# Eydcao/BSMS-GNN

Hardware: AMD Instinct MI355X
Metric: rollout steps/sec (1-step fwd+bwd) on airfoil mesh, batch=8 (higher is better)
Workload: dtype f32; 1 GPU; airfoil-like Delaunay mesh, 5233 nodes, 5 bi-stride levels, D=128, hidden_layer=3, batch 8 per GPU (global 8), consistent mesh; global_batch=8, parallelism=dp1, trainable_params=1917827

## Files before the change

### bsms-gnn_amd/build.py

```python
import hashlib
import os
import subprocess
import sys
from concurrent.futures import ThreadPoolExecutor

HERE = os.path.dirname(os.path.abspath(__file__))
CSRC = os.path.join(HERE, "csrc")
OBJ = os.path.join(HERE, "_build")
LIB = os.path.join(HERE, "libbsms_hip.so")
SOURCES = ["plan.hip", "rowsum.hip", "chain.hip", "chain_d32.hip", "chain_d64.hip", "chain_d96.hip", "chain_d128.hip", "chain_d160.hip", "chain_d192.hip", "chain_d224.hip",
           "chain_d256.hip", "efuse.hip", "efwd.hip", "wgrad.hip", "gmp.hip", "mlp.hip", "bsgmp.hip", "optim.hip", "hierarchy.hip", "sim.hip", "posgrad.hip", "batch.hip", "errsum.hip"]
HEADERS = ["common.h", "chain.h", "host_orch.h", "gmp_block.h", "chain_dev.h", "chain_kernels.h", "chain_edge.h", "chain_launch.h", os.path.join("..", "..", "include", "bsms_hip.h")]
FLAGS = ["--offload-arch=gfx950", "-O3", "-std=c++17", "-fPIC", "-Wall", "-Wno-unused-function"]
if os.environ.get("BSMS_EXPERIMENTS") == "1":
    FLAGS.append("-DBSMS_EXPERIMENTS")


def _hipcc():
    for c in (os.environ.get("HIPCC"), "/opt/rocm/bin/hipcc", "hipcc"):
        if c and (os.path.isabs(c) and os.path.exists(c) or not os.path.isabs(c)):
            return c
    raise RuntimeError("hipcc not found")


def _digest():
    h = hashlib.sha256((" ".join(FLAGS) + os.environ.get("BSMS_CHAIN_FLAGS", "")).encode())
    for f in SOURCES + HEADERS:
        with open(os.path.join(CSRC, f), "rb") as fh:
            h.update(fh.read())
    return h.hexdigest()


def build(force=False, verbose=True):
    os.makedirs(OBJ, exist_ok=True)
    stamp = os.path.join(OBJ, "stamp")
    digest = _digest()
    if not force and os.path.exists(LIB) and os.path.exists(stamp) and open(stamp).read() == digest:
        return LIB
    hipcc = _hipcc()

    def compile_one(src):
        obj = os.path.join(OBJ, os.path.basename(src).replace(".hip", ".o"))
        extra = ["-ffp-contract=off"] if src in ("rowsum.hip", "sim.hip", "batch.hip", "errsum.hip") else []
        if src.startswith("chain") and os.environ.get("BSMS_CHAIN_FLAGS"):
            extra += os.environ["BSMS_CHAIN_FLAGS"].split()
        cmd = [hipcc, *FLAGS, *extra, "-c", os.path.join(CSRC, src), "-o", obj]
        r = subprocess.run(cmd, capture_output=True, text=True)
        if r.returncode != 0:
            raise RuntimeError(f"hipcc failed on {src}:\n{r.stdout}\n{r.stderr}")
        if verbose and r.stderr.strip():
            print(r.stderr, file=sys.stderr)
        return obj

    with ThreadPoolExecutor(max_workers=len(SOURCES)) as ex:
        objs = list(ex.map(compile_one, SOURCES))
    r = subprocess.run([hipcc, "--offload-arch=gfx950", "-shared", "-fPIC", "-o", LIB, *objs], capture_output=True, text=True)
    if r.returncode != 0:
        raise RuntimeError(f"link failed:\n{r.stdout}\n{r.stderr}")
    with open(stamp, "w") as fh:
        fh.write(digest)
    if verbose:
        print(f"built {LIB} ({os.path.getsize(LIB) / 1e6:.1f} MB)")
    return LIB


# ... 44 lines not shown
```

### bsms-gnn_amd/csrc/chain.h

```cpp
#pragma once
#include "common.h"

namespace bsms {

constexpr int kMaxStages = 8;
constexpr int kComputeWaves = 4;
constexpr int kTileRows = kComputeWaves * 16;
constexpr int kChainThreads = (kComputeWaves + 1) * 64;
constexpr int kChainMaxThreads = 8 * 64;
constexpr int kChunkHdrFloats = 256;
constexpr size_t mask_words_per_row(int64_t D) { return size_t(4) * size_t((D + 127) / 128); }
constexpr int kPadRows = 2 * kTileRows;
constexpr size_t pad_rows(size_t rows) { return (rows + kPadRows - 1) / kPadRows * kPadRows + 2 * kPadRows; }
constexpr size_t act_floats(size_t rows, int64_t D) { return pad_rows(rows) * (size_t(D) + mask_words_per_row(D)); }
constexpr int fiber_ld(int64_t p) { return p + 1 <= 4 ? 4 : 8; }
constexpr int kScaleSlot = 255;
constexpr size_t pack_floats(int64_t D) { return size_t(D / 32) * (kChunkHdrFloats + size_t(D / 16) * 512); }

enum ChainIn { IN_ROWS = 0, IN_ROWS2 = 1, IN_SMALL = 2, IN_EDGE = 3 };
enum ChainOut { OUT_LN = 0, OUT_PLAIN = 1, OUT_SMALL = 2, OUT_PLAIN2 = 3 };
enum GradIn { G_ROWS_LN = 0, G_EDGE_LN = 1, G_SMALL = 2 };
enum GradFirst { F_NONE = 0, F_HEADS1 = 1, F_HEADS2 = 2 };

struct ChainFwdArgs {
  int64_t R;
  int ntiles;
  const float* x;
  const float* x2;
  int K0;
  const float* w0t;
  const float* bias_in;
  float* store_in;
  const int32_t *src, *dst;
  int32_t E, N;
  const float *Ps, *Pd;
  const float* pos;
  int64_t pos_bstride;
  int p;
  float* fiber_out;
  int nstage;
  const float4* wp[kMaxStages];
  const float4* wp0b;
  float* store[kMaxStages];
  float* y;
  float* y2;
  float* yln;
  float* rstd;
  const float* resid;
  const float* resid2;
  int accumulate;
  const float* wout;
  const float* bout;
  int C;
  unsigned long long* timing;
  int bf16;
  int store_mode;
  int out_mode;
  int nseq;
  const float4* wseq[kMaxStages + 2];
  int nload;
  int nring;
  float* amax[kMaxStages + 1];
};

struct ChainBwdArgs {
  int64_t R;
  int ntiles;
  const float* dy;
  const float* yln;
  const float* rstd;
  const int32_t* dst;
  int32_t E, N;
  const float* wout;
  int C;
  const float* mask_in;
  int nstage;
  const float4* wpt[kMaxStages];
  const float* mask[kMaxStages];
  float* gstore[kMaxStages + 1];
  const float4 *wh0, *wh1;
  float *dx, *dx2;
  const float* dres;
  int store_mode;
  int bf16;
  int nseq;
  const float4* wseq[kMaxStages + 2];
  int nload;
  int nring;
  float* gmax[kMaxStages + 1];
  int ablate;
};

enum PackKind { PACK_FRAG = 0, PACK_FRAG_T = 1, PACK_TRANSPOSE = 2, PACK_ROWS_BF16 = 3 };
struct PackDesc {
  const float* W;
  const float* bias;
  float* dst;
  int ld, row0, col0;
  int N, K;
  int kind;
  int bf16;
  int mate;
};
constexpr int kMaxPack = 40;
constexpr int kBoundWidth = 8192;
constexpr int kBoundSlots = 32;
struct PackTable {
  int n;
  PackDesc d[kMaxPack];
  float* zero;
};
int launch_prepack(const PackTable& t, hipStream_t s);

struct PackGroup {
  std::vector<PackDesc> descs;
  std::vector<float*> zeros;
  int biggest = 0;
  void* dev = nullptr;
  int device = -1;
};
void pack_group_append(PackGroup& g, const PackTable& t);
int launch_prepack_group(PackGroup& g, hipStream_t s);
int pack_group_open(bsms_pack_group_t* group, const char* who, PackGroup** g);

int launch_chain_fwd(int D, int in_mode, int out_mode, const ChainFwdArgs& a, hipStream_t s);
int launch_chain_bwd(int D, int gin_mode, int first_mode, const ChainBwdArgs& a, hipStream_t s);
template <int NB>
int launch_chain_fwd_nb(int in_mode, int out_mode, const ChainFwdArgs& a, hipStream_t s);
template <int NB>
int launch_chain_bwd_nb(int gin_mode, int first_mode, const ChainBwdArgs& a, hipStream_t s);

struct WgradJob {
  const float* G;
  const float* A;
  float* dW;
  float* db;
  int64_t R;
  int ldg, lda, ldw, col0;
  int bf16;
  const float *g_bound, *a_bound;
  float g_mul, a_mul;
// ... 82 lines not shown
```

### bsms-gnn_amd/csrc/chain_dev.h

```cpp
#pragma once
#include "chain.h"

using namespace bsms;

namespace {


using f32x4 = __attribute__((ext_vector_type(4))) float;
#ifndef BSMS_CHAIN_WPE
#define BSMS_CHAIN_WPE 4
#endif
constexpr int kPL = 2;


using f32x2 = __attribute__((ext_vector_type(2))) float;
using bf16x2 = __attribute__((ext_vector_type(2))) __bf16;
__device__ __forceinline__ unsigned pk_bf16(float lo, float hi) {
  const f32x2 v = {lo, hi};
  return __builtin_bit_cast(unsigned, __builtin_convertvector(v, bf16x2));
}
__device__ __forceinline__ float bf16_lo(unsigned u) { return __uint_as_float(u << 16); }
__device__ __forceinline__ float bf16_hi(unsigned u) { return __uint_as_float(u & 0xffff0000u); }

template <int NB>
// ... 129 lines not shown
      const int e = 32 * w + k;
      m = __builtin_amdgcn_alignbit(m, 0u - __float_as_uint(v[e >> 2][e & 3]), 31);
    }
    bits[w] = m;
  }
}

template <int NB>
__device__ __forceinline__ void load_features(f32x4 (&v)[NB], const float* vec, int g) {
  load_rows<NB>(v, vec, g);
}

__device__ __forceinline__ float group_sum(float s) {
  s += __shfl_xor(s, 16, 64);
  s += __shfl_xor(s, 32, 64);
  return s;
}

template <int NB>
__device__ __forceinline__ float row_sum(const f32x4 (&v)[NB]) {
  float s = 0.f;
#pragma unroll
  for (int t = 0; t < NB; ++t) s += (v[t][0] + v[t][1]) + (v[t][2] + v[t][3]);
  return group_sum(s);
}

template <int NB, int PL = kPL>
struct Ring {
  static constexpr int D = NB * 16;
  static constexpr int NCH = NB / 2;
  static constexpr int CHF = kChunkHdrFloats + NB * 256 * PL;
  static constexpr int CH4 = CHF / 4;
  static constexpr int PER = CHF / 256;
  static constexpr int SIDE_FLOATS = 8 * D;
  static constexpr int PRE_FLOATS = SIDE_FLOATS + 256;
  static constexpr int PRE4 = PRE_FLOATS / 4;
  static constexpr size_t lds_bytes(int nr) { return (size_t(PRE_FLOATS) + size_t(nr) * CHF) * sizeof(float); }
  static_assert(CHF % 256 == 0 && PER < 64, "chunk = whole LDS-DMA instructions, countable by vmcnt");
  static_assert(NB % 2 == 0, "K blocks are pairs of 16-feature blocks");
};

__device__ __forceinline__ void lds_barrier() { asm volatile("s_waitcnt lgkmcnt(0)\n\ts_barrier" ::: "memory"); }

__device__ __forceinline__ void glds16(const void* gsrc, unsigned lds_dst) {
  unsigned keep;
  asm volatile("s_mov_b32 %0, m0\n\ts_mov_b32 m0, %2\n\ts_nop 0\n\tglobal_load_lds_dwordx4 %1, off\n\ts_mov_b32 m0, %0"
               : "=&s"(keep) : "v"(gsrc), "s"(lds_dst) : "memory");
}

struct Slot { int i, nr; };

template <int NB, int PL, int NL, int LI>
__device__ __forceinline__ void loader_run(const float4* const* wseq, int nseq, float4* lds, int lane, int ntiles, int nr,
                                           const float* side = nullptr) {
  using R = Ring<NB, PL>;
  constexpr int MINE = (R::PER - LI + NL - 1) / NL;
  __builtin_amdgcn_s_setprio(3);
  const unsigned pre0 = __builtin_amdgcn_readfirstlane((unsigned)(uintptr_t)lds);
  const unsigned lds0 = pre0 + unsigned(R::PRE_FLOATS * sizeof(float));
  if (side) {
    if (LI == 0) {
      const unsigned dst = pre0;
#pragma unroll
      for (int i = 0; i < R::SIDE_FLOATS / 256; ++i) glds16(reinterpret_cast<const float4*>(side) + i * 64 + lane, dst + i * 1024);
    }
    asm volatile("s_waitcnt vmcnt(0)\n\ts_barrier" ::: "memory");
  }
  const int my_tiles = (ntiles - int(blockIdx.x) + int(gridDim.x) - 1) / int(gridDim.x);
  const int per_tile = nseq * R::NCH, total = my_tiles * per_tile;
  int is = 0, ic = 0, islot = 0;
  auto issue = [&]() {
    const float4* src = wseq[is] + size_t(ic) * R::CH4 + lane;
    const unsigned dst = lds0 + unsigned(islot) * unsigned(R::CHF * sizeof(float));
#pragma unroll
    for (int i = 0; i < MINE; ++i) glds16(src + (LI + i * NL) * 64, dst + (LI + i * NL) * 1024);
    if (++ic == R::NCH) { ic = 0; if (++is == nseq) is = 0; }
    if (++islot == nr) islot = 0;
  };
  const int ahead = nr - 1;
  for (int j = 0; j < ahead && j < total; ++j) issue();
  for (int j = 0; j < total; ++j) {
    const int younger = min(ahead - 1, total - 1 - j);
    switch (younger) {
      case 0: asm volatile("s_waitcnt vmcnt(0)" ::: "memory"); break;
      case 1: asm volatile("s_waitcnt vmcnt(%0)" ::"n"(MINE) : "memory"); break;
      case 2: asm volatile("s_waitcnt vmcnt(%0)" ::"n"(2 * MINE <= 63 ? 2 * MINE : 63) : "memory"); break;
      case 3: asm volatile("s_waitcnt vmcnt(%0)" ::"n"(3 * MINE <= 63 ? 3 * MINE : 63) : "memory"); break;
      default: asm volatile("s_waitcnt vmcnt(%0)" ::"n"(4 * MINE <= 63 ? 4 * MINE : 63) : "memory"); break;
    }
    asm volatile("s_barrier" ::: "memory");
    if (j + ahead < total) issue();
  }
}
template <int NB, int PL = kPL>
__device__ __forceinline__ void loader_dispatch(int nl, int li, const float4* const* wseq, int nseq, float4* lds, int lane, int ntiles,
                                                int nr, const float* side = nullptr) {
  if (nl == 1) loader_run<NB, PL, 1, 0>(wseq, nseq, lds, lane, ntiles, nr, side);
  else if (nl == 2) { if (li == 0) loader_run<NB, PL, 2, 0>(wseq, nseq, lds, lane, ntiles, nr, side); else loader_run<NB, PL, 2, 1>(wseq, nseq, lds, lane, ntiles, nr, side); }
  else { if (li == 0) loader_run<NB, PL, 3, 0>(wseq, nseq, lds, lane, ntiles, nr, side); else if (li == 1) loader_run<NB, PL, 3, 1>(wseq, nseq, lds, lane, ntiles, nr, side);
         else loader_run<NB, PL, 3, 2>(wseq, nseq, lds, lane, ntiles, nr, side); }
}

using u32x4 = __attribute__((ext_vector_type(4))) unsigned;
using bf16x8 = __attribute__((ext_vector_type(8))) __bf16;
using f16x8 = __attribute__((ext_vector_type(8))) _Float16;

template <int NB>
__device__ __forceinline__ void split_block(const f32x4 (&act)[NB], int kb2, float s, u32x4& bh, u32x4& bl) {
#pragma unroll
  for (int v = 0; v < 4; ++v) {
    unsigned h, l;
    split_h2(act[2 * kb2 + (v >> 1)][2 * (v & 1)], act[2 * kb2 + (v >> 1)][2 * (v & 1) + 1], s, h, l);
    bh[v] = h;
    bl[v] = l;
  }
}

template <int NB>
__device__ __forceinline__ void round_block(const f32x4 (&act)[NB], int kb2, u32x4& bh) {
#pragma unroll
  for (int v = 0; v < 4; ++v) bh[v] = pk_bf16(act[2 * kb2 + (v >> 1)][2 * (v & 1)], act[2 * kb2 + (v >> 1)][2 * (v & 1) + 1]);
}

__device__ __forceinline__ f32x4 mma_bf(const float4& a, const u32x4& b, f32x4 c) {
  return __builtin_amdgcn_mfma_f32_16x16x32_bf16(__builtin_bit_cast(bf16x8, a), __builtin_bit_cast(bf16x8, b), c, 0, 0, 0);
}
__device__ __forceinline__ f32x4 mma(const float4& a, const u32x4& b, f32x4 c) {
  return __builtin_amdgcn_mfma_f32_16x16x32_f16(__builtin_bit_cast(f16x8, a), __builtin_bit_cast(f16x8, b), c, 0, 0, 0);
}

template <int NB>
__device__ __forceinline__ float row_amax(const f32x4 (&v)[NB]) {
  float m = 0.f;
#pragma unroll
  for (int t = 0; t < NB; ++t) {
    m = fmaxf(fmaxf(m, fabsf(v[t][0])), fabsf(v[t][1]));
    m = fmaxf(fmaxf(m, fabsf(v[t][2])), fabsf(v[t][3]));
  }
  m = fmaxf(m, __shfl_xor(m, 16, 64));
  return fmaxf(m, __shfl_xor(m, 32, 64));
}

__device__ __forceinline__ bool any_slot(float* const (&slots)[kMaxStages + 1]) {
  bool any = false;
#pragma unroll
  for (int k = 0; k <= kMaxStages; ++k) any |= slots[k] != nullptr;
  return any;
}
template <int NB>
__device__ __forceinline__ unsigned* bound_row(float4* lds, int wave, int lane, bool wanted) {
  if (!wanted) return nullptr;
  unsigned* row = reinterpret_cast<unsigned*>(reinterpret_cast<float*>(lds) + Ring<NB>::SIDE_FLOATS) + wave * 16;
  if (lane < 16) row[lane] = 0u;
// ... 267 lines not shown
```

### bsms-gnn_amd/csrc/chain_edge.h

```cpp
#pragma once
#include "chain_dev.h"

namespace {

struct PairOff { unsigned a, b; };
template <int NB>
__device__ __forceinline__ PairOff pair_offsets(int64_t row, int lane) {
  constexpr int D = NB * 16;
  const bool hi = (lane & 8) != 0;
  const int64_t rowA = row - (lane & 8);
  return PairOff{unsigned((rowA * D + 4 * (lane >> 4) + (hi ? 16 : 0)) * 4), unsigned(((rowA + 8) * D + 4 * (lane >> 4) + (hi ? 0 : 16)) * 4)};
}
template <int NB>
__device__ __forceinline__ void store_pair_nt(const f32x4 (&v)[NB], float* base, PairOff off, int lane, int t) {
  using i32x4 = __attribute__((ext_vector_type(4))) int;
  const bool hi = (lane & 8) != 0;
  const i32x4 own = __builtin_bit_cast(i32x4, v[t + 1]);
  i32x4 got;
#pragma unroll
  for (int r = 0; r < 4; ++r) got[r] = __builtin_amdgcn_update_dpp(own[r], own[r], 0x128, 0xf, 0xf, false);
  const f32x4 x = __builtin_bit_cast(f32x4, got);
  const f32x4 dA = hi ? x : v[t], dB = hi ? v[t] : x;
  char* b = reinterpret_cast<char*>(base) + 64 * t;
  __builtin_nontemporal_store(dA, reinterpret_cast<f32x4*>(b + off.a));
// ... 179 lines not shown
    float4 f0 = body[0], f1 = body[2 * 64];
    if (c == 0) fw = int(__float_as_uint(reinterpret_cast<const float*>(cur)[kScaleSlot]) >> 23);
    const int cb = c & 1;
    int islot = 0;
    auto pair = [&](int t, int rb, const float4& a0, const float4& a1, const unsigned (&piece)[4], bool first) {
      acc[rb][t] = mma(a0, vec4(piece), (ZERO && first && c == 0) ? zero : acc[rb][t]);
      acc[rb][t + 1] = mma(a1, vec4(piece), (ZERO && first && c == 0) ? zero : acc[rb][t + 1]);
      const int s = (islot * NSTEP + NSLOT - 1) / NSLOT;
      if (s < NSTEP && s * NSLOT / NSTEP == islot)
        valu_step<NB, RB, SAVE, MASK>(s, c, act, pc, st, rs, mword, store_base, bits_base, off, moff, lane);
      ++islot;
      __builtin_amdgcn_sched_barrier(0);
    };
    __builtin_amdgcn_sched_barrier(0);
#pragma unroll
    for (int t = 0; t < NB; t += 2) {
      float4 n0 = body[(t * 2 + 1) * 64], n1 = body[(t * 2 + 3) * 64];
#pragma unroll
      for (int rb = 0; rb < RB; ++rb) pair(t, rb, f0, f1, pc[rb][cb].l, true);
#pragma unroll
      for (int rb = 0; rb < RB; ++rb) pair(t, rb, f0, f1, pc[rb][cb].h, false);
      f0 = n0;
      f1 = n1;
      if (t + 2 < NB) {
        n0 = body[((t + 2) * 2) * 64];
        n1 = body[((t + 2) * 2 + 2) * 64];
      }
#pragma unroll
      for (int rb = 0; rb < RB; ++rb) pair(t, rb, f0, f1, pc[rb][cb].h, false);
      f0 = n0;
      f1 = n1;
    }
    if (FIN != 0 && c == Rg::NCH - 1) {
#pragma unroll
      for (int rb = 0; rb < RB; ++rb) finish_stage<NB, FIN == 2>(acc[rb], rs[rb].E, fw, reinterpret_cast<const float*>(cur), lane);
    }
  }
}

template <int NB, int RB>
struct EdgeTile {
  static constexpr int rows = kTileRows * RB;
  static constexpr int waves_per_eu = (NB * RB <= 8) ? 4 : 2;
  static constexpr int resident = (NB * RB <= 8) ? 2 : 1;
};

template <int NB, int RB, int SAVE, bool LONE = false>
__global__ __launch_bounds__(kChainMaxThreads) __attribute__((amdgpu_waves_per_eu(LONE ? 2 : EdgeTile<NB, RB>::waves_per_eu)))
void k_edge_fwd(ChainFwdArgs a) {
  constexpr int D = NB * 16;
  extern __shared__ __attribute__((aligned(16))) float4 lds[];
  const int tid = threadIdx.x, lane = tid & 63, wave = tid >> 6, lg = lane >> 4;
  const int cw = int(blockDim.x >> 6) - a.nload, tile_rows = 16 * RB * cw;
  if (wave >= cw) {
    loader_dispatch<NB>(a.nload, wave - cw, a.wseq, a.nseq, lds, lane, a.ntiles, a.nring, a.w0t);
    return;
  }
  const float rcpE = 1.f / float(a.E);
  auto fetch_endpoints = [&](int tile, int (&i)[RB], int (&j)[RB], int (&b)[RB]) {
#pragma unroll
    for (int rb = 0; rb < RB; ++rb) {
      const int64_t r = int64_t(tile) * tile_rows + wave * (16 * RB) + rb * 16 + (lane & 15);
      const EdgeRef e = edge_ref(unsigned(r < a.R ? r : 0), unsigned(a.E), rcpE);
      i[rb] = a.src[e.q];
      j[rb] = a.dst[e.q];
      b[rb] = e.b;
    }
  };
  int ni[RB], nj[RB], nbat[RB];
  fetch_endpoints(blockIdx.x, ni, nj, nbat);
  lds_barrier();
  const float* w0t = reinterpret_cast<const float*>(lds);
  Slot slot{0, a.nring};
  float4* const ring = lds + Ring<NB>::PRE4;
  unsigned* brow = bound_row<NB>(lds, wave, lane, any_slot(a.amax));
  for (int tile = blockIdx.x; tile < a.ntiles; tile += gridDim.x) {
    int64_t row[RB];
    PairOff off[RB];
    unsigned moff[RB];
    f32x4 act[RB][NB], acc[RB][NB];
    float pi[RB][7], pj[RB][7];
#ifdef BSMS_EXPERIMENTS
    int stamp_i = 0;
    unsigned long long waited = 0;
    auto stamp = [&]() { if (a.timing && tid == 0 && stamp_i < 16) a.timing[int64_t(tile) * 16 + stamp_i++] = __builtin_amdgcn_s_memtime(); };
#else
    auto stamp = [] {};
#endif
    stamp();
#pragma unroll
    for (int rb = 0; rb < RB; ++rb) {
      row[rb] = int64_t(tile) * tile_rows + wave * (16 * RB) + rb * 16 + (lane & 15);
      off[rb] = pair_offsets<NB>(wave * (16 * RB) + rb * 16 + (lane & 15), lane);
      moff[rb] = unsigned(((wave * (16 * RB) + rb * 16 + (lane & 15)) * (4 * mask_words<NB>()) + lg * mask_words<NB>()) * 4);
      const int i = ni[rb], j = nj[rb], b = nbat[rb];
      load_rows<NB>(act[rb], a.Ps + (int64_t(b) * a.N + i) * D, lg);
      load_rows<NB>(acc[rb], a.Pd + (int64_t(b) * a.N + j) * D, lg);
      const float* pb = a.pos + b * a.pos_bstride;
      if (a.p == 2) {
        const float2 xi = *reinterpret_cast<const float2*>(pb + int64_t(i) * 2), xj = *reinterpret_cast<const float2*>(pb + int64_t(j) * 2);
        pi[rb][0] = xi.x; pi[rb][1] = xi.y; pj[rb][0] = xj.x; pj[rb][1] = xj.y;
#pragma unroll
        for (int c = 2; c < 7; ++c) pi[rb][c] = pj[rb][c] = 0.f;
      } else {
#pragma unroll
        for (int c = 0; c < 7; ++c) {
          const int cc = c < a.p ? c : 0;
          pi[rb][c] = pb[int64_t(i) * a.p + cc];
          pj[rb][c] = pb[int64_t(j) * a.p + cc];
        }
      }
    }
    if (tile + int(gridDim.x) < a.ntiles) fetch_endpoints(tile + gridDim.x, ni, nj, nbat);
    __builtin_amdgcn_sched_barrier(0);
    stamp();
#pragma unroll
    for (int rb = 0; rb < RB; ++rb) {
#pragma unroll
      for (int t = 0; t < NB; ++t) act[rb][t] += acc[rb][t];
      float n2 = 0.f;
#pragma unroll
      for (int c = 0; c < 7; ++c)
        if (c < a.p) {
          const float rel = pi[rb][c] - pj[rb][c];
          n2 = fmaf(rel, rel, n2);
          axpy_features<NB>(act[rb], w0t + c * D, rel, lg);
        }
      const float nrm = sqrtf(n2);
      axpy_features<NB>(act[rb], w0t + a.p * D, nrm, lg);
      relu_into<NB>(act[rb], act[rb]);
      if (a.fiber_out && row[rb] < a.R && lg == 0) {
        float f[8];
#pragma unroll
        for (int c = 0; c < 7; ++c) f[c] = c < a.p ? pi[rb][c] - pj[rb][c] : (c == a.p ? nrm : 0.f);
        f[7] = a.p == 7 ? nrm : 0.f;
        const int ld = fiber_ld(a.p);
        float4* dst = reinterpret_cast<float4*>(a.fiber_out + row[rb] * ld);
        dst[0] = make_float4(f[0], f[1], f[2], f[3]);
        if (ld == 8) dst[1] = make_float4(f[4], f[5], f[6], f[7]);
      }
    }
    float* pending = a.store_in;
    stamp();
    for (int l = 0; l < a.nstage; ++l) {
      float* st_tile = SAVE ? pending + int64_t(tile) * (tile_rows * D) : nullptr;
      unsigned* bits_tile = SAVE ? reinterpret_cast<unsigned*>(pending + pad_rows(a.R) * D) + int64_t(tile) * (tile_rows * 4 * mask_words<NB>()) : nullptr;
#ifdef BSMS_EXPERIMENTS
      stage_rb<NB, RB, SAVE, true, true, 2, LONE>(acc, act, ring, slot, lane, st_tile, bits_tile, off, moff, brow, l, nullptr, a.timing ? &waited : nullptr);
#else
      stage_rb<NB, RB, SAVE, true, true, 2, LONE>(acc, act, ring, slot, lane, st_tile, bits_tile, off, moff, brow, l);
#endif
      stamp();
      if (l + 1 < a.nstage) {
#pragma unroll
        for (int rb = 0; rb < RB; ++rb) relu_into<NB>(act[rb], acc[rb]);
        pending = a.store[l];
      }
    }
#pragma unroll
    for (int rb = 0; rb < RB; ++rb) {
      const float mean = row_sum<NB>(acc[rb]) * (1.f / D);
      float ss = 0.f;
#pragma unroll
      for (int t = 0; t < NB; ++t)
#pragma unroll
        for (int r = 0; r < 4; ++r) {
          acc[rb][t][r] -= mean;
          ss = fmaf(acc[rb][t][r], acc[rb][t][r], ss);
        }
      ss = group_sum(ss);
      const float rstd = 1.f / sqrtf(ss * (1.f / D) + 1e-5f);
#pragma unroll
      for (int t = 0; t < NB; ++t)
#pragma unroll
        for (int r = 0; r < 4; ++r) acc[rb][t][r] *= rstd;
      const int64_t roff = row[rb] < a.R ? row[rb] * D : -1;
      store_rows<NB, false>(acc[rb], a.yln, roff, lg);
      if (a.rstd && roff >= 0 && lg == 0) a.rstd[row[rb]] = rstd;
      store_rows<NB, false>(acc[rb], a.y, roff, lg, a.out_mode);
    }
    stamp();
#ifdef BSMS_EXPERIMENTS
    if (a.timing && tid == 0) a.timing[int64_t(tile) * 16 + 11] = waited;
#endif
  }
  if (SAVE) flush_bounds(a.amax, kMaxStages + 1, brow, wave, lane);
}

template <int NB, int RB, bool LONE = false, bool STORE = true>
__global__ __launch_bounds__(kChainMaxThreads) __attribute__((amdgpu_waves_per_eu(LONE ? 2 : EdgeTile<NB, RB>::waves_per_eu)))
void k_edge_bwd(ChainBwdArgs a) {
  constexpr int D = NB * 16, W = mask_words<NB>();
  extern __shared__ __attribute__((aligned(16))) float4 lds[];
  const int tid = threadIdx.x, lane = tid & 63, wave = tid >> 6, lg = lane >> 4;
  const int cw = int(blockDim.x >> 6) - a.nload, tile_rows = 16 * RB * cw;
  if (wave >= cw) {
    loader_dispatch<NB>(a.nload, wave - cw, a.wseq, a.nseq, lds, lane, a.ntiles, a.nring);
    return;
  }
  const float rcpE = 1.f / float(a.E);
  auto fetch_targets = [&](int tile, int64_t (&node)[RB]) {
#pragma unroll
    for (int rb = 0; rb < RB; ++rb) {
      const int64_t r = int64_t(tile) * tile_rows + wave * (16 * RB) + rb * 16 + (lane & 15);
      const EdgeRef e = edge_ref(unsigned(r < a.R ? r : 0), unsigned(a.E), rcpE);
      node[rb] = int64_t(e.b) * a.N + a.dst[e.q];
    }
  };
  int64_t nnode[RB];
  fetch_targets(blockIdx.x, nnode);
  Slot slot{0, a.nring};
  float4* const ring = lds + Ring<NB>::PRE4;
  unsigned* brow = bound_row<NB>(lds, wave, lane, any_slot(a.gmax));
  for (int tile = blockIdx.x; tile < a.ntiles; tile += gridDim.x) {
    int64_t row[RB], rowc[RB];
    PairOff off[RB];
    unsigned moff[RB];
    f32x4 g[RB][NB], acc[RB][NB];
    float rs[RB];
#pragma unroll
    for (int rb = 0; rb < RB; ++rb) {
      row[rb] = int64_t(tile) * tile_rows + wave * (16 * RB) + rb * 16 + (lane & 15);
      rowc[rb] = row[rb] < a.R ? row[rb] : 0;
      off[rb] = pair_offsets<NB>(wave * (16 * RB) + rb * 16 + (lane & 15), lane);
      moff[rb] = 0;
      load_rows<NB>(g[rb], a.dy + nnode[rb] * D, lg);
      load_rows<NB>(acc[rb], a.yln + rowc[rb] * D, lg);
      rs[rb] = a.rstd[rowc[rb]];
    }
    if (tile + int(gridDim.x) < a.ntiles) fetch_targets(tile + gridDim.x, nnode);
    __builtin_amdgcn_sched_barrier(0);
#pragma unroll
    for (int rb = 0; rb < RB; ++rb) {
      const float m1 = row_sum<NB>(g[rb]) * (1.f / D);
      float s2 = 0.f;
#pragma unroll
      for (int t = 0; t < NB; ++t)
#pragma unroll
        for (int r = 0; r < 4; ++r) s2 = fmaf(g[rb][t][r], acc[rb][t][r], s2);
      s2 = group_sum(s2);
      const float m2 = s2 * (1.f / D);
#pragma unroll
      for (int t = 0; t < NB; ++t)
#pragma unroll
        for (int r = 0; r < 4; ++r) g[rb][t][r] = rs[rb] * (g[rb][t][r] - m1 - acc[rb][t][r] * m2);
    }
    float* pending = a.gstore[0];
    for (int k = 0; k < a.nstage; ++k) {
      unsigned mbits[RB][W];
#pragma unroll
      for (int rb = 0; rb < RB; ++rb)
#pragma unroll
        for (int w = 0; w < W; ++w)
          mbits[rb][w] = reinterpret_cast<const unsigned*>(a.mask[k] + pad_rows(a.R) * D)[rowc[rb] * (4 * W) + lg * W + w];
#ifdef BSMS_EXPERIMENTS
      float* const gtile = STORE ? pending + int64_t(a.ablate ? 0 : tile) * (tile_rows * D) : nullptr;
#else
      float* const gtile = STORE ? pending + int64_t(tile) * (tile_rows * D) : nullptr;
#endif
      stage_rb<NB, RB, STORE ? 1 : 0, false, true, 1, LONE>(acc, g, ring, slot, lane, gtile, nullptr, off, moff, brow, k);
#pragma unroll
      for (int rb = 0; rb < RB; ++rb)
#pragma unroll
        for (int t = 0; t < NB; ++t)
#pragma unroll
          for (int r = 0; r < 4; ++r) {
            const int keep = __builtin_amdgcn_sbfe((int)mbits[rb][(4 * t + r) >> 5], (4 * t + r) & 31, 1);
            g[rb][t][r] = __uint_as_float(__float_as_uint(acc[rb][t][r]) & (unsigned)keep);
          }
      pending = a.gstore[k + 1];
    }
#pragma unroll
    for (int rb = 0; rb < RB; ++rb) {
      if (a.gmax[a.nstage]) note_amax(brow, a.nstage, row_amax<NB>(g[rb]), lane);
      store_rows<NB, false>(g[rb], pending, row[rb] < a.R ? row[rb] * D : -1, lg);
    }
  }
  flush_bounds(a.gmax, kMaxStages + 1, brow, wave, lane);
}

}
```

### bsms-gnn_amd/csrc/chain_launch.h

```cpp
#pragma once
#include <algorithm>
#include <cstdlib>

#include "chain_edge.h"
#include "chain_kernels.h"

namespace {

template <int NB>
constexpr int resident_per_cu() { return NB <= 4 ? 4 : NB == 8 ? 2 : 1; }

template <int NB>
int chain_compute_waves(int64_t R) {
  const int cus = device_cu_count();
  const int64_t slots = int64_t(cus) * resident_per_cu<NB>();
  if (resident_per_cu<NB>() >= 4 || ceil_div(R, kTileRows) <= slots) return kComputeWaves;
  const int64_t need = ceil_div(R, slots * 16);
  return need <= 7 ? (int)need : kComputeWaves;
}

template <int NB>
unsigned persistent_grid(int64_t ntiles) {
  const int cus = device_cu_count();
  return (unsigned)std::min<int64_t>(ntiles, int64_t(cus) * resident_per_cu<NB>());
}

inline int knob(const char* name, int dflt) {
#ifdef BSMS_EXPERIMENTS
  const char* e = getenv(name);
  return e ? atoi(e) : dflt;
#else
  (void)name;
  return dflt;
#endif
}

inline int edge_rb_mode() {
#ifdef BSMS_EXPERIMENTS
  static const int m = [] { const char* e = getenv("BSMS_EDGE_RB"); return e ? atoi(e) : -1; }();
  return m;
#else
  return -1;
#endif
}

template <int NB>
int edge_compute_waves() {
  static const int cw = NB >= 16 ? knob("BSMS_EDGE_CW16", 7) : knob("BSMS_EDGE_CW", 7);
  return cw;
}
template <int NB, int RB>
int pick_edge_waves(int64_t R) {
  const int fixed = edge_compute_waves<NB>();
#ifdef BSMS_EXPERIMENTS
  if (getenv(NB >= 16 ? "BSMS_EDGE_CW16" : "BSMS_EDGE_CW") || getenv("BSMS_EDGE_CW_FIXED")) return fixed;
#endif
  const double slope = (NB >= 16 ? 0.25 : 0.53) * RB;
  const int64_t slots = int64_t(device_cu_count()) * EdgeTile<NB, RB>::resident;
  auto cost_of = [&](int cw) {
    const int64_t tiles = ceil_div(R, int64_t(16) * RB * cw);
    const int64_t per = ceil_div(tiles, std::min<int64_t>(tiles, slots));
    return double(per) * (1.0 + slope * cw);
  };
  int best = fixed;
  double best_cost = cost_of(fixed) * 0.92;
  for (int cw = 6; cw >= 4; --cw) {
    const double cost = cost_of(cw);
    if (cost < best_cost * (1.0 - 1e-9)) { best_cost = cost; best = cw; }
  }
  return best;
}
template <int NB>
int edge_loader_waves() {
  static const int nl = NB >= 16 ? knob("BSMS_EDGE_NL16", 1) : knob("BSMS_EDGE_NL", 1);
  return nl;
}
inline int chain_loader_waves() {
  static const int nl = knob("BSMS_CHAIN_NL", 1);
  return nl;
}

template <int NB, int PL = kPL>
int max_ring() { return (int)std::min<size_t>(6, (size_t(160) * 1024 - Ring<NB, PL>::PRE_FLOATS * sizeof(float)) / (Ring<NB, PL>::CHF * sizeof(float))); }
template <int NB, int PL = kPL>
void pick_stream(int64_t ntiles, int cw, int nload_default, int& nload, int& nring) {
  static const int deep = knob("BSMS_RING_DEEP", 6), lone_nl = knob("BSMS_LONE_NL", 2), shared = knob("BSMS_RING", 3);
  nload = std::max(1, std::min(nload_default, 8 - cw));
  nring = std::min(shared, max_ring<NB, PL>());
  if (ntiles <= device_cu_count()) {
    nload = std::max(nload, std::min(lone_nl, 8 - cw));
    nring = std::min(deep, max_ring<NB, PL>());
  }
  const int mine = (Ring<NB, PL>::PER + nload - 1) / nload;
  while (nring > 3 && (nring - 2) * mine > 63) --nring;
}

template <int NB>
size_t ring_lds_max() { return Ring<NB>::lds_bytes(max_ring<NB>()); }

template <int NB, int RB, int SAVE>
int launch_edge_fwd_t(ChainFwdArgs& a, hipStream_t s) {
  const int cw = pick_edge_waves<NB, RB>(a.R);
  a.ntiles = (int)ceil_div(a.R, 16 * RB * cw);
  pick_stream<NB>(a.ntiles, cw, edge_loader_waves<NB>(), a.nload, a.nring);
  const unsigned grid = (unsigned)std::min<int64_t>(a.ntiles, int64_t(device_cu_count()) * EdgeTile<NB, RB>::resident);
  const unsigned threads = (cw + a.nload) * 64;
  const size_t lds = Ring<NB>::lds_bytes(a.nring);
  static const int lone = knob("BSMS_EDGE_LONE", 1);
  if (lone && a.ntiles <= device_cu_count() && !a.timing)
    return launch_dyn_lds<k_edge_fwd<NB, RB, SAVE, true>>("edge_fwd", "single-round build", grid, threads, lds, ring_lds_max<NB>(), a, s);
  return launch_dyn_lds<k_edge_fwd<NB, RB, SAVE>>("edge_fwd", nullptr, grid, threads, lds, ring_lds_max<NB>(), a, s);
}

template <int NB>
bool launch_edge_fwd(ChainFwdArgs& a, hipStream_t s, int& rc) {
  if (a.bf16 || a.nstage < 1 || a.store_mode != 1 || a.resid || a.resid2 || edge_rb_mode() == 0 || a.R >= (int64_t(1) << 31)) return false;
  const bool save = a.store_in != nullptr;
  for (int l = 0; l + 1 < a.nstage; ++l)
    if ((a.store[l] != nullptr) != save) return false;
  constexpr int RBIG = NB == 8 ? 2 : 1;
  const int64_t cus = device_cu_count(), rows1 = 16 * edge_compute_waves<NB>();
  bool big = RBIG == 2 && a.R >= cus * rows1 && ceil_div(a.R, rows1) <= cus * EdgeTile<NB, 1>::resident;
  if (edge_rb_mode() > 0) big = RBIG == 2 && edge_rb_mode() == 2;
  if (big) rc = save ? launch_edge_fwd_t<NB, RBIG, 1>(a, s) : launch_edge_fwd_t<NB, RBIG, 0>(a, s);
  else rc = save ? launch_edge_fwd_t<NB, 1, 1>(a, s) : launch_edge_fwd_t<NB, 1, 0>(a, s);
  return true;
}

template <int NB, int RB, bool STORE>
int launch_edge_bwd_t(ChainBwdArgs& a, hipStream_t s) {
  const int cw = pick_edge_waves<NB, RB>(a.R);
  a.ntiles = (int)ceil_div(a.R, 16 * RB * cw);
  pick_stream<NB>(a.ntiles, cw, edge_loader_waves<NB>(), a.nload, a.nring);
  const unsigned grid = (unsigned)std::min<int64_t>(a.ntiles, int64_t(device_cu_count()) * EdgeTile<NB, RB>::resident);
  const unsigned threads = (cw + a.nload) * 64;
  const size_t lds = Ring<NB>::lds_bytes(a.nring);
  static const int lone = knob("BSMS_EDGE_LONE", 1);
  if (lone && a.ntiles <= device_cu_count())
    return launch_dyn_lds<k_edge_bwd<NB, RB, true, STORE>>("edge_bwd", STORE ? "single-round build" : "single-round no-store build", grid, threads, lds, ring_lds_max<NB>(), a, s);
  return launch_dyn_lds<k_edge_bwd<NB, RB, false, STORE>>("edge_bwd", STORE ? nullptr : "no-store build", grid, threads, lds, ring_lds_max<NB>(), a, s);
}

template <int NB>
bool launch_edge_bwd(ChainBwdArgs& a, hipStream_t s, int& rc) {
  if (a.bf16 || a.nstage < 1 || a.store_mode != 1 || edge_rb_mode() == 0 || a.R >= (int64_t(1) << 31)) return false;
  if (!a.gstore[a.nstage]) return false;
  const bool store = a.gstore[0] != nullptr;
  for (int k = 0; k < a.nstage; ++k)
    if ((a.gstore[k] != nullptr) != store || !a.mask[k]) return false;
  constexpr int RBIG = NB == 8 ? 2 : 1;
  bool big = RBIG == 2 && a.R >= int64_t(device_cu_count()) * 16 * edge_compute_waves<NB>();
  if (edge_rb_mode() > 0) big = RBIG == 2 && edge_rb_mode() == 2;
  if (store) rc = big ? launch_edge_bwd_t<NB, RBIG, true>(a, s) : launch_edge_bwd_t<NB, 1, true>(a, s);
  else rc = big ? launch_edge_bwd_t<NB, RBIG, false>(a, s) : launch_edge_bwd_t<NB, 1, false>(a, s);
  return true;
}

template <int NB>
int bf_edge_waves(int64_t R) {
  static const int forced = knob("BSMS_BFEDGE_CW", 0);
  if (forced > 0) return forced;
  return R > int64_t(device_cu_count()) * resident_per_cu<NB>() * 16 * kComputeWaves ? 7 : kComputeWaves;
}

template <int NB, int IN, int OUT>
int launch_fwd_t(const ChainFwdArgs& a0, hipStream_t s) {
  ChainFwdArgs a = a0;
  a.nseq = 0;
  for (int l = 0; l < a.nstage; ++l) {
    a.wseq[a.nseq++] = a.wp[l];
    if (IN == IN_ROWS2 && l == 0) a.wseq[a.nseq++] = a.wp0b;
  }
  if constexpr ((NB == 8 || NB == 16) && IN == IN_EDGE && OUT == OUT_LN) {
    int rc = BSMS_OK;
    if (launch_edge_fwd<NB>(a, s, rc)) return rc;
  }
  if constexpr (NB == 8 && (IN == IN_ROWS || IN == IN_ROWS2 || IN == IN_SMALL)) {
    static const int fs_rows = knob("BSMS_FS_ROWS", kFsMaxRows);
    if (!a.bf16 && a.R <= fs_rows && a.nseq >= 1 && a.nseq <= kMaxStages + 1) {
      hipLaunchKernelGGL((k_fs_fwd<IN, OUT>), dim3((unsigned)ceil_div(a.R, 16)), dim3(256), 0, s, a);
      BSMS_LAUNCH_CHECK();
      return BSMS_OK;
    }
  }
  int cw = (IN == IN_EDGE) ? bf_edge_waves<NB>(a.R) : chain_compute_waves<NB>(a.R);
  a.ntiles = (int)ceil_div(a.R, 16 * cw);
  bool rows2_lone = false;
// ... 107 lines not shown
```

Before: 196.3 steps/s.

## Balance edge-kernel tail tiles across blocks by splitting leftover row blocks

Edge forward and backward kernels now map work in two parts: full rounds of tiles strided over the grid, plus a remainder of 16*RB-row blocks spread evenly across all blocks. Each block's leftover share runs with only some of its compute waves active, and the idle waves keep the ring barriers in step. This targets tail imbalance when the tile count is not a multiple of the resident slots. The wave-count cost model also changes to match the new mapping. The extra branching and the partial-wave barrier loop add complexity and risk of sync mismatch.

```diff
diff --git a/bsms-gnn_amd/build.py b/bsms-gnn_amd/build.py
--- a/bsms-gnn_amd/build.py
+++ b/bsms-gnn_amd/build.py
@@ -10,7 +10,7 @@
 LIB = os.path.join(HERE, "libbsms_hip.so")
 SOURCES = ["plan.hip", "rowsum.hip", "chain.hip", "chain_d32.hip", "chain_d64.hip", "chain_d96.hip", "chain_d128.hip", "chain_d160.hip", "chain_d192.hip", "chain_d224.hip",
            "chain_d256.hip", "efuse.hip", "efwd.hip", "wgrad.hip", "gmp.hip", "mlp.hip", "bsgmp.hip", "optim.hip", "hierarchy.hip", "sim.hip", "posgrad.hip", "batch.hip", "errsum.hip"]
-HEADERS = ["common.h", "chain.h", "host_orch.h", "gmp_block.h", "chain_dev.h", "chain_kernels.h", "chain_edge.h", "chain_launch.h", os.path.join("..", "..", "include", "bsms_hip.h")]
+HEADERS = ["common.h", "chain.h", "host_orch.h", "gmp_block.h", "chain_dev.h", "chain_kernels.h", "chain_edge.h", "chain_launch.h", "edge_balance.h", os.path.join("..", "..", "include", "bsms_hip.h")]
 FLAGS = ["--offload-arch=gfx950", "-O3", "-std=c++17", "-fPIC", "-Wall", "-Wno-unused-function"]
 if os.environ.get("BSMS_EXPERIMENTS") == "1":
     FLAGS.append("-DBSMS_EXPERIMENTS")
diff --git a/bsms-gnn_amd/csrc/chain.h b/bsms-gnn_amd/csrc/chain.h
--- a/bsms-gnn_amd/csrc/chain.h
+++ b/bsms-gnn_amd/csrc/chain.h
@@ -1,5 +1,6 @@
 #pragma once
 #include "common.h"
+#include "edge_balance.h"
 
 namespace bsms {
 
@@ -60,6 +61,7 @@
   const float4* wseq[kMaxStages + 2];
   int nload;
   int nring;
+  EdgeBalance bal;
   float* amax[kMaxStages + 1];
 };
 
@@ -87,6 +89,7 @@
   const float4* wseq[kMaxStages + 2];
   int nload;
   int nring;
+  EdgeBalance bal;
   float* gmax[kMaxStages + 1];
   int ablate;
 };
diff --git a/bsms-gnn_amd/csrc/chain_dev.h b/bsms-gnn_amd/csrc/chain_dev.h
--- a/bsms-gnn_amd/csrc/chain_dev.h
+++ b/bsms-gnn_amd/csrc/chain_dev.h
@@ -205,7 +205,7 @@
 
 template <int NB, int PL, int NL, int LI>
 __device__ __forceinline__ void loader_run(const float4* const* wseq, int nseq, float4* lds, int lane, int ntiles, int nr,
-                                           const float* side = nullptr) {
+                                           const float* side = nullptr, int given_tiles = -1) {
   using R = Ring<NB, PL>;
   constexpr int MINE = (R::PER - LI + NL - 1) / NL;
   __builtin_amdgcn_s_setprio(3);
@@ -219,7 +219,7 @@
     }
     asm volatile("s_waitcnt vmcnt(0)\n\ts_barrier" ::: "memory");
   }
-  const int my_tiles = (ntiles - int(blockIdx.x) + int(gridDim.x) - 1) / int(gridDim.x);
+  const int my_tiles = given_tiles >= 0 ? given_tiles : (ntiles - int(blockIdx.x) + int(gridDim.x) - 1) / int(gridDim.x);
   const int per_tile = nseq * R::NCH, total = my_tiles * per_tile;
   int is = 0, ic = 0, islot = 0;
   auto issue = [&]() {
@@ -247,11 +247,11 @@
 }
 template <int NB, int PL = kPL>
 __device__ __forceinline__ void loader_dispatch(int nl, int li, const float4* const* wseq, int nseq, float4* lds, int lane, int ntiles,
-                                                int nr, const float* side = nullptr) {
-  if (nl == 1) loader_run<NB, PL, 1, 0>(wseq, nseq, lds, lane, ntiles, nr, side);
-  else if (nl == 2) { if (li == 0) loader_run<NB, PL, 2, 0>(wseq, nseq, lds, lane, ntiles, nr, side); else loader_run<NB, PL, 2, 1>(wseq, nseq, lds, lane, ntiles, nr, side); }
-  else { if (li == 0) loader_run<NB, PL, 3, 0>(wseq, nseq, lds, lane, ntiles, nr, side); else if (li == 1) loader_run<NB, PL, 3, 1>(wseq, nseq, lds, lane, ntiles, nr, side);
-         else loader_run<NB, PL, 3, 2>(wseq, nseq, lds, lane, ntiles, nr, side); }
+                                                int nr, const float* side = nullptr, int given_tiles = -1) {
+  if (nl == 1) loader_run<NB, PL, 1, 0>(wseq, nseq, lds, lane, ntiles, nr, side, given_tiles);
+  else if (nl == 2) { if (li == 0) loader_run<NB, PL, 2, 0>(wseq, nseq, lds, lane, ntiles, nr, side, given_tiles); else loader_run<NB, PL, 2, 1>(wseq, nseq, lds, lane, ntiles, nr, side, given_tiles); }
+  else { if (li == 0) loader_run<NB, PL, 3, 0>(wseq, nseq, lds, lane, ntiles, nr, side, given_tiles); else if (li == 1) loader_run<NB, PL, 3, 1>(wseq, nseq, lds, lane, ntiles, nr, side, given_tiles);
+         else loader_run<NB, PL, 3, 2>(wseq, nseq, lds, lane, ntiles, nr, side, given_tiles); }
 }
 
 using u32x4 = __attribute__((ext_vector_type(4))) unsigned;
diff --git a/bsms-gnn_amd/csrc/chain_edge.h b/bsms-gnn_amd/csrc/chain_edge.h
--- a/bsms-gnn_amd/csrc/chain_edge.h
+++ b/bsms-gnn_amd/csrc/chain_edge.h
@@ -255,15 +255,20 @@
   extern __shared__ __attribute__((aligned(16))) float4 lds[];
   const int tid = threadIdx.x, lane = tid & 63, wave = tid >> 6, lg = lane >> 4;
   const int cw = int(blockDim.x >> 6) - a.nload, tile_rows = 16 * RB * cw;
+  const EdgeShare sh = edge_share(a.bal, int(blockIdx.x), int(gridDim.x));
+  const int my_tiles = sh.tiles();
   if (wave >= cw) {
-    loader_dispatch<NB>(a.nload, wave - cw, a.wseq, a.nseq, lds, lane, a.ntiles, a.nring, a.w0t);
+    loader_dispatch<NB>(a.nload, wave - cw, a.wseq, a.nseq, lds, lane, a.ntiles, a.nring, a.w0t, my_tiles);
     return;
   }
   const float rcpE = 1.f / float(a.E);
-  auto fetch_endpoints = [&](int tile, int (&i)[RB], int (&j)[RB], int (&b)[RB]) {
-#pragma unroll
-    for (int rb = 0; rb < RB; ++rb) {
-      const int64_t r = int64_t(tile) * tile_rows + wave * (16 * RB) + rb * 16 + (lane & 15);
+  auto tile_row0 = [&](int it) -> int64_t {
+    return it < sh.nfull ? (int64_t(blockIdx.x) + int64_t(it) * gridDim.x) * tile_rows : int64_t(sh.left_first) * (16 * RB);
+  };
+  auto fetch_endpoints = [&](int64_t row0, int (&i)[RB], int (&j)[RB], int (&b)[RB]) {
+#pragma unroll
+    for (int rb = 0; rb < RB; ++rb) {
+      const int64_t r = row0 + wave * (16 * RB) + rb * 16 + (lane & 15);
       const EdgeRef e = edge_ref(unsigned(r < a.R ? r : 0), unsigned(a.E), rcpE);
       i[rb] = a.src[e.q];
       j[rb] = a.dst[e.q];
@@ -271,19 +276,28 @@
     }
   };
   int ni[RB], nj[RB], nbat[RB];
-  fetch_endpoints(blockIdx.x, ni, nj, nbat);
+  fetch_endpoints(tile_row0(0), ni, nj, nbat);
   lds_barrier();
   const float* w0t = reinterpret_cast<const float*>(lds);
   Slot slot{0, a.nring};
   float4* const ring = lds + Ring<NB>::PRE4;
   unsigned* brow = bound_row<NB>(lds, wave, lane, any_slot(a.amax));
-  for (int tile = blockIdx.x; tile < a.ntiles; tile += gridDim.x) {
+  for (int it = 0; it < my_tiles; ++it) {
+    if (!LONE && it >= sh.nfull && wave >= sh.nleft) {
+      for (int c = 0; c < a.nstage * Ring<NB>::NCH; ++c) {
+        lds_barrier();
+        if (++slot.i == slot.nr) slot.i = 0;
+      }
+      break;
+    }
+    const int64_t row0 = tile_row0(it);
     int64_t row[RB];
     PairOff off[RB];
     unsigned moff[RB];
     f32x4 act[RB][NB], acc[RB][NB];
     float pi[RB][7], pj[RB][7];
 #ifdef BSMS_EXPERIMENTS
+    const int tile = int(blockIdx.x) + it * int(gridDim.x);
     int stamp_i = 0;
     unsigned long long waited = 0;
     auto stamp = [&]() { if (a.timing && tid == 0 && stamp_i < 16) a.timing[int64_t(tile) * 16 + stamp_i++] = __builtin_amdgcn_s_memtime(); };
@@ -293,7 +307,7 @@
     stamp();
 #pragma unroll
     for (int rb = 0; rb < RB; ++rb) {
-      row[rb] = int64_t(tile) * tile_rows + wave * (16 * RB) + rb * 16 + (lane & 15);
+      row[rb] = row0 + wave * (16 * RB) + rb * 16 + (lane & 15);
       off[rb] = pair_offsets<NB>(wave * (16 * RB) + rb * 16 + (lane & 15), lane);
       moff[rb] = unsigned(((wave * (16 * RB) + rb * 16 + (lane & 15)) * (4 * mask_words<NB>()) + lg * mask_words<NB>()) * 4);
       const int i = ni[rb], j = nj[rb], b = nbat[rb];
@@ -314,7 +328,7 @@
         }
       }
     }
-    if (tile + int(gridDim.x) < a.ntiles) fetch_endpoints(tile + gridDim.x, ni, nj, nbat);
+    if (it + 1 < my_tiles) fetch_endpoints(tile_row0(it + 1), ni, nj, nbat);
     __builtin_amdgcn_sched_barrier(0);
     stamp();
 #pragma unroll
@@ -346,8 +360,8 @@
     float* pending = a.store_in;
     stamp();
     for (int l = 0; l < a.nstage; ++l) {
-      float* st_tile = SAVE ? pending + int64_t(tile) * (tile_rows * D) : nullptr;
-      unsigned* bits_tile = SAVE ? reinterpret_cast<unsigned*>(pending + pad_rows(a.R) * D) + int64_t(tile) * (tile_rows * 4 * mask_words<NB>()) : nullptr;
+      float* st_tile = SAVE ? pending + row0 * D : nullptr;
+      unsigned* bits_tile = SAVE ? reinterpret_cast<unsigned*>(pending + pad_rows(a.R) * D) + row0 * (4 * mask_words<NB>()) : nullptr;
 #ifdef BSMS_EXPERIMENTS
       stage_rb<NB, RB, SAVE, true, true, 2, LONE>(acc, act, ring, slot, lane, st_tile, bits_tile, off, moff, brow, l, nullptr, a.timing ? &waited : nullptr);
 #else
@@ -397,25 +411,38 @@
   extern __shared__ __attribute__((aligned(16))) float4 lds[];
   const int tid = threadIdx.x, lane = tid & 63, wave = tid >> 6, lg = lane >> 4;
   const int cw = int(blockDim.x >> 6) - a.nload, tile_rows = 16 * RB * cw;
+  const EdgeShare sh = edge_share(a.bal, int(blockIdx.x), int(gridDim.x));
+  const int my_tiles = sh.tiles();
   if (wave >= cw) {
-    loader_dispatch<NB>(a.nload, wave - cw, a.wseq, a.nseq, lds, lane, a.ntiles, a.nring);
+    loader_dispatch<NB>(a.nload, wave - cw, a.wseq, a.nseq, lds, lane, a.ntiles, a.nring, nullptr, my_tiles);
     return;
   }
   const float rcpE = 1.f / float(a.E);
-  auto fetch_targets = [&](int tile, int64_t (&node)[RB]) {
-#pragma unroll
-    for (int rb = 0; rb < RB; ++rb) {
-      const int64_t r = int64_t(tile) * tile_rows + wave * (16 * RB) + rb * 16 + (lane & 15);
+  auto tile_row0 = [&](int it) -> int64_t {
+    return it < sh.nfull ? (int64_t(blockIdx.x) + int64_t(it) * gridDim.x) * tile_rows : int64_t(sh.left_first) * (16 * RB);
+  };
+  auto fetch_targets = [&](int64_t row0, int64_t (&node)[RB]) {
+#pragma unroll
+    for (int rb = 0; rb < RB; ++rb) {
+      const int64_t r = row0 + wave * (16 * RB) + rb * 16 + (lane & 15);
       const EdgeRef e = edge_ref(unsigned(r < a.R ? r : 0), unsigned(a.E), rcpE);
       node[rb] = int64_t(e.b) * a.N + a.dst[e.q];
     }
   };
   int64_t nnode[RB];
-  fetch_targets(blockIdx.x, nnode);
+  fetch_targets(tile_row0(0), nnode);
   Slot slot{0, a.nring};
   float4* const ring = lds + Ring<NB>::PRE4;
   unsigned* brow = bound_row<NB>(lds, wave, lane, any_slot(a.gmax));
-  for (int tile = blockIdx.x; tile < a.ntiles; tile += gridDim.x) {
+  for (int it = 0; it < my_tiles; ++it) {
+    if (!LONE && it >= sh.nfull && wave >= sh.nleft) {
+      for (int c = 0; c < a.nstage * Ring<NB>::NCH; ++c) {
+        lds_barrier();
+        if (++slot.i == slot.nr) slot.i = 0;
+      }
+      break;
+    }
+    const int64_t row0 = tile_row0(it);
     int64_t row[RB], rowc[RB];
     PairOff off[RB];
     unsigned moff[RB];
@@ -423,7 +450,7 @@
     float rs[RB];
 #pragma unroll
     for (int rb = 0; rb < RB; ++rb) {
-      row[rb] = int64_t(tile) * tile_rows + wave * (16 * RB) + rb * 16 + (lane & 15);
+      row[rb] = row0 + wave * (16 * RB) + rb * 16 + (lane & 15);
       rowc[rb] = row[rb] < a.R ? row[rb] : 0;
       off[rb] = pair_offsets<NB>(wave * (16 * RB) + rb * 16 + (lane & 15), lane);
       moff[rb] = 0;
@@ -431,7 +458,7 @@
       load_rows<NB>(acc[rb], a.yln + rowc[rb] * D, lg);
       rs[rb] = a.rstd[rowc[rb]];
     }
-    if (tile + int(gridDim.x) < a.ntiles) fetch_targets(tile + gridDim.x, nnode);
+    if (it + 1 < my_tiles) fetch_targets(tile_row0(it + 1), nnode);
     __builtin_amdgcn_sched_barrier(0);
 #pragma unroll
     for (int rb = 0; rb < RB; ++rb) {
@@ -457,9 +484,9 @@
         for (int w = 0; w < W; ++w)
           mbits[rb][w] = reinterpret_cast<const unsigned*>(a.mask[k] + pad_rows(a.R) * D)[rowc[rb] * (4 * W) + lg * W + w];
 #ifdef BSMS_EXPERIMENTS
-      float* const gtile = STORE ? pending + int64_t(a.ablate ? 0 : tile) * (tile_rows * D) : nullptr;
+      float* const gtile = STORE ? pending + (a.ablate ? 0 : row0) * D : nullptr;
 #else
-      float* const gtile = STORE ? pending + int64_t(tile) * (tile_rows * D) : nullptr;
+      float* const gtile = STORE ? pending + row0 * D : nullptr;
 #endif
       stage_rb<NB, RB, STORE ? 1 : 0, false, true, 1, LONE>(acc, g, ring, slot, lane, gtile, nullptr, off, moff, brow, k);
 #pragma unroll
diff --git a/bsms-gnn_amd/csrc/chain_launch.h b/bsms-gnn_amd/csrc/chain_launch.h
--- a/bsms-gnn_amd/csrc/chain_launch.h
+++ b/bsms-gnn_amd/csrc/chain_launch.h
@@ -49,19 +49,20 @@
   static const int cw = NB >= 16 ? knob("BSMS_EDGE_CW16", 7) : knob("BSMS_EDGE_CW", 7);
   return cw;
 }
+constexpr int kEdgeBalanceDefault = 1;
+inline bool edge_balance_on() {
+  static const int on = knob("BSMS_EDGE_BALANCE", kEdgeBalanceDefault);
+  return on != 0;
+}
 template <int NB, int RB>
-int pick_edge_waves(int64_t R) {
+int pick_edge_waves(int64_t R, bool balance) {
   const int fixed = edge_compute_waves<NB>();
 #ifdef BSMS_EXPERIMENTS
   if (getenv(NB >= 16 ? "BSMS_EDGE_CW16" : "BSMS_EDGE_CW") || getenv("BSMS_EDGE_CW_FIXED")) return fixed;
 #endif
   const double slope = (NB >= 16 ? 0.25 : 0.53) * RB;
   const int64_t slots = int64_t(device_cu_count()) * EdgeTile<NB, RB>::resident;
-  auto cost_of = [&](int cw) {
-    const int64_t tiles = ceil_div(R, int64_t(16) * RB * cw);
-    const int64_t per = ceil_div(tiles, std::min<int64_t>(tiles, slots));
-    return double(per) * (1.0 + slope * cw);
-  };
+  auto cost_of = [&](int cw) { return edge_cost(edge_map(R, RB, cw, slots, balance), cw, slope); };
   int best = fixed;
   double best_cost = cost_of(fixed) * 0.92;
   for (int cw = 6; cw >= 4; --cw) {
@@ -100,10 +101,13 @@
 
 template <int NB, int RB, int SAVE>
 int launch_edge_fwd_t(ChainFwdArgs& a, hipStream_t s) {
-  const int cw = pick_edge_waves<NB, RB>(a.R);
-  a.ntiles = (int)ceil_div(a.R, 16 * RB * cw);
+  const bool balance = edge_balance_on() && !a.timing;
+  const int cw = pick_edge_waves<NB, RB>(a.R, balance);
+  const EdgeMap map = edge_map(a.R, RB, cw, int64_t(device_cu_count()) * EdgeTile<NB, RB>::resident, balance);
+  a.ntiles = (int)map.tiles;
+  a.bal = map.bal;
   pick_stream<NB>(a.ntiles, cw, edge_loader_waves<NB>(), a.nload, a.nring);
-  const unsigned grid = (unsigned)std::min<int64_t>(a.ntiles, int64_t(device_cu_count()) * EdgeTile<NB, RB>::resident);
+  const unsigned grid = map.grid;
   const unsigned threads = (cw + a.nload) * 64;
   const size_t lds = Ring<NB>::lds_bytes(a.nring);
   static const int lone = knob("BSMS_EDGE_LONE", 1);
@@ -129,10 +133,13 @@
 
 template <int NB, int RB, bool STORE>
 int launch_edge_bwd_t(ChainBwdArgs& a, hipStream_t s) {
-  const int cw = pick_edge_waves<NB, RB>(a.R);
-  a.ntiles = (int)ceil_div(a.R, 16 * RB * cw);
+  const bool balance = edge_balance_on();
+  const int cw = pick_edge_waves<NB, RB>(a.R, balance);
+  const EdgeMap map = edge_map(a.R, RB, cw, int64_t(device_cu_count()) * EdgeTile<NB, RB>::resident, balance);
+  a.ntiles = (int)map.tiles;
+  a.bal = map.bal;
   pick_stream<NB>(a.ntiles, cw, edge_loader_waves<NB>(), a.nload, a.nring);
-  const unsigned grid = (unsigned)std::min<int64_t>(a.ntiles, int64_t(device_cu_count()) * EdgeTile<NB, RB>::resident);
+  const unsigned grid = map.grid;
   const unsigned threads = (cw + a.nload) * 64;
   const size_t lds = Ring<NB>::lds_bytes(a.nring);
   static const int lone = knob("BSMS_EDGE_LONE", 1);
diff --git a/bsms-gnn_amd/csrc/edge_balance.h b/bsms-gnn_amd/csrc/edge_balance.h
--- /dev/null
+++ b/bsms-gnn_amd/csrc/edge_balance.h
@@ -0,0 +1,67 @@
+#pragma once
+#include <cstdint>
+
+#if defined(__HIPCC__) || defined(__CUDACC__)
+#define BSMS_HOST_DEVICE __host__ __device__
+#else
+#define BSMS_HOST_DEVICE
+#endif
+
+namespace bsms {
+
+struct EdgeBalance {
+  int full_tiles;
+  int left_start;
+  int left_q;
+  int left_r;
+};
+
+struct EdgeShare {
+  int nfull;
+  int nleft;
+  int left_first;
+  BSMS_HOST_DEVICE int tiles() const { return nfull + (nleft > 0 ? 1 : 0); }
+};
+BSMS_HOST_DEVICE inline EdgeShare edge_share(const EdgeBalance& b, int g, int grid) {
+  EdgeShare s;
+  s.nfull = g < b.full_tiles ? (b.full_tiles - g + grid - 1) / grid : 0;
+  s.nleft = b.left_q + (g < b.left_r ? 1 : 0);
+  s.left_first = b.left_start + g * b.left_q + (g < b.left_r ? g : b.left_r);
+  return s;
+}
+
+struct EdgeMap {
+  int64_t tiles;
+  int64_t blocks;
+  unsigned grid;
+  int64_t rounds;
+  int64_t left_blocks;
+  EdgeBalance bal;
+};
+
+inline EdgeMap edge_map(int64_t R, int RB, int cw, int64_t slots, bool balance = true) {
+  EdgeMap m;
+  const int64_t brows = int64_t(16) * RB;
+  m.blocks = (R + brows - 1) / brows;
+  m.tiles = (R + brows * cw - 1) / (brows * cw);
+  m.grid = unsigned(m.tiles < slots ? m.tiles : slots);
+  if (!balance || m.tiles <= slots) {
+    m.rounds = m.grid ? (m.tiles + m.grid - 1) / m.grid : 0;
+    m.left_blocks = 0;
+    m.bal = EdgeBalance{int(m.tiles), 0, 0, 0};
+    return m;
+  }
+  const int64_t per_round = int64_t(m.grid) * cw;
+  m.rounds = m.blocks / per_round;
+  m.left_blocks = m.blocks - m.rounds * per_round;
+  m.bal = EdgeBalance{int(m.rounds * m.grid), int(m.rounds * per_round), int(m.left_blocks / m.grid), int(m.left_blocks % m.grid)};
+  return m;
+}
+
+inline double edge_cost(const EdgeMap& m, int cw, double slope) {
+  double c = double(m.rounds) * (1.0 + slope * cw);
+  if (m.left_blocks > 0) c += 1.0 + slope * double((m.left_blocks + m.grid - 1) / m.grid);
+  return c;
+}
+
+}
diff --git a/profiles/edge_levels.py b/profiles/edge_levels.py
--- /dev/null
+++ b/profiles/edge_levels.py
@@ -0,0 +1,22 @@
+#!/usr/bin/env python3
+import csv
+import re
+import sys
+
+trace = sorted(csv.DictReader(open(sys.argv[1])), key=lambda r: int(r["Start_Timestamp"]))
+traced = int(sys.argv[2]) if len(sys.argv) > 2 else 25
+keep = int(sys.argv[3]) if len(sys.argv) > 3 else 20
+for fam in ("k_edge_fwd", "k_edge_bwd"):
+    rows = [r for r in trace if fam + "<" in r["Kernel_Name"]]
+    per = len(rows) // traced
+    rows = rows[-keep * per:]
+    total = 0.0
+    for pos in range(per):
+        rs = rows[pos::per]
+        d = [(int(r["End_Timestamp"]) - int(r["Start_Timestamp"])) / 1e3 for r in rs]
+        targs = re.search(fam + r"<([^>]*)>", rs[0]["Kernel_Name"]).group(1)
+        wg = int(rs[0]["Workgroup_Size"]) if "Workgroup_Size" in rs[0] else int(rs[0]["Workgroup_Size_X"])
+        grid = int(rs[0]["Grid_Size"]) if "Grid_Size" in rs[0] else int(rs[0]["Grid_Size_X"])
+        total += sum(d) / len(d)
+        print(f"{fam} #{pos:2d} <{targs:18s}> grid {grid // wg:4d} x {wg // 64 - 1} waves  mean {sum(d) / len(d):7.1f} us  min {min(d):7.1f} us")
+    print(f"{fam} total {total:8.1f} us per step over {per} launches")
```

Result: no change. 198.0 steps/s, median of 6 (+0.9%).
